# refresh-bio/colord

Measured on AMD Instinct MI355X. Metric: input Gbases/s + archive size vs ref, ONT 50 Gb at 1/2/4/8 MI355X, higher is better.
Workload: dtype u64

## Files before the change

colord_amd/_native.py:

```python
from __future__ import annotations
import ctypes as C
import os

os.environ.setdefault("GPU_MAX_HW_QUEUES", "32")
_HERE = os.path.dirname(os.path.abspath(__file__))
LIB_PATH = os.environ.get("COLORD_HIP_LIBRARY") or os.path.join(_HERE, "libcolord_hip.so")

CL_OK, CL_E_INVALID, CL_E_HIP, CL_E_CAPACITY, CL_E_NOMEM, CL_E_UNSUPPORTED = 0, -1, -2, -3, -4, -5


class ColordHipError(RuntimeError):
    def __init__(self, status, msg):
        super().__init__(f"colord_hip error {status}: {msg}")
        self.status = status


class QualParams(C.Structure):
    _fields_ = [("mode", C.c_int32), ("source", C.c_int32), ("level", C.c_int32), ("n_fwd", C.c_uint32), ("fwd", C.c_uint32 * 8),
                ("n_rev", C.c_uint32), ("rev", C.c_uint32 * 8)]


class KmerStats(C.Structure):
    _fields_ = [("n_reads", C.c_uint64), ("tot_kmers", C.c_uint64), ("n_unique", C.c_uint64),
                ("n_unique_counted", C.c_uint64), ("total_count_filtered", C.c_uint64)]
# ... 46 lines not shown
    "cl_kmer_count_filter": (C.c_int32, [_P, _P, C.c_uint64, C.c_uint32, C.c_uint32, C.c_uint32, C.POINTER(_P), C.POINTER(KmerStats)]),
    "cl_kmer_set_create": (C.c_int32, [_P, _P, _P, C.c_uint64, C.c_uint32, C.POINTER(_P)]),
    "cl_kmer_set_free": (None, [_P]),
    "cl_kmer_set_size": (C.c_uint64, [_P]),
    "cl_kmer_set_keys": (_P, [_P]),
    "cl_kmer_set_counts": (_P, [_P]),
    "cl_kmer_set_check": (C.c_int32, [_P, _P, _P, C.c_uint64, _P]),
    "cl_accepted_kmers": (C.c_int32, [_P, _P, _P, C.c_uint32, C.c_uint32, C.POINTER(_P)]),
    "cl_kmer_lists_free": (None, [_P]),
    "cl_kmer_lists_reads": (C.c_uint32, [_P]),
    "cl_kmer_lists_total": (C.c_uint64, [_P]),
    "cl_kmer_lists_offsets": (_P, [_P]),
    "cl_kmer_lists_kmers": (_P, [_P]),
    "cl_kmer_lists_ids": (_P, [_P]),
    "cl_kmer_lists_pos": (_P, [_P]),
    "cl_ref_accept": (C.c_int32, [C.c_uint32, C.c_uint32, C.c_uint32, C.c_double, _P]),
    "cl_index_build": (C.c_int32, [_P, _P, _P, _P, C.c_uint32, C.c_uint32, C.POINTER(_P)]),
    "cl_index_entries_of": (C.c_int32, [_P, _P, _P, C.c_uint32, _P, _P, C.c_uint64, C.POINTER(C.c_uint64), _P, C.POINTER(C.c_uint32)]),
    "cl_index_build_pairs": (C.c_int32, [_P, _P, _P, _P, C.c_uint64, _P, C.c_uint32, C.c_uint32, C.c_uint32, C.c_uint32, C.POINTER(_P)]),
    "cl_index_free": (None, [_P]),
    "cl_index_n_refs": (C.c_uint32, [_P]),
    "cl_index_entries": (C.c_uint64, [_P]),
    "cl_index_ref_rank": (_P, [_P]),
    "cl_candidates": (C.c_int32, [_P, _P, _P, C.c_uint32, _P, _P, _P]),
    "cl_candidates_common": (C.c_int32, [_P, _P, _P, C.c_uint32, _P, _P, _P, _P, C.c_uint64, C.POINTER(C.c_uint64)]),
    "cl_qual_coder_create": (C.c_int32, [_P, C.POINTER(QualParams), C.POINTER(_P)]),
    "cl_qual_coder_ctx": (_P, [_P]),
    "cl_qual_coder_free": (None, [_P]),
    "cl_qual_encode": (C.c_int32, [_P, _P, _P, _P, _P, _P, _P, C.c_uint32, _P, C.c_uint64, _P, C.POINTER(C.c_uint64)]),
    "cl_anchor_candidates": (C.c_int32, [_P, _P, _P, _P, _P, C.c_uint32, C.c_uint32, C.c_double, C.c_double, C.c_double, C.c_uint32, C.POINTER(_P)]),
    "cl_anchor_candidates_hifi": (C.c_int32, [_P, _P, _P, _P, _P, C.c_uint32, C.c_uint32, C.c_double, C.c_double, C.c_double, C.c_uint32, C.c_uint32, C.c_uint32, _P, _P, C.POINTER(_P)]),
    "cl_anchors_free": (None, [_P]),
    "cl_anchors_total": (C.c_uint64, [_P]),
    "cl_anchors_n_cands": (_P, [_P]),
    "cl_anchors_cands": (_P, [_P]),
    "cl_anchors_cand_offsets": (_P, [_P]),
    "cl_anchors_data": (_P, [_P]),
    "cl_encode_plain": (C.c_int32, [_P, _P, _P, C.c_uint64, _P, _P, C.POINTER(C.c_uint64)]),
    "cl_reads_select": (C.c_int32, [_P, _P, _P, C.POINTER(_P)]),
    "cl_reads_from_arena": (C.c_int32, [_P, _P, _P, _P, C.c_uint32, C.POINTER(_P)]),
    "cl_estimator_logs": (C.c_int32, [_P, _P, _P, C.c_uint64, _P]),
    "cl_es_flags": (C.c_int32, [_P, _P, _P, _P, _P, _P]),
    "cl_id_coder_create": (C.c_int32, [C.c_int32, C.POINTER(_P)]),
    "cl_id_coder_free": (None, [_P]),
    "cl_id_coder_error": (C.c_char_p, [_P]),
    "cl_id_encode_part": (C.c_int32, [_P, _P, _P, _P, C.c_uint32, _P, C.c_uint64, C.POINTER(C.c_uint64)]),
    "cl_compress_shard": (C.c_int32, [_P, C.POINTER(CompressParams), _P, _P, _P, _P, C.c_uint32, _P, C.c_uint32, _P, _P, _P, C.c_uint64, _P, _P, C.c_uint64, _P,
                                      C.POINTER(CompressInfo)]),
    "cl_candidates_at": (C.c_int32, [_P, _P, _P, _P, C.c_uint32, _P, _P, _P]),
    "cl_compressor_create": (C.c_int32, [_P, _P, C.POINTER(CompressParams), C.POINTER(QualParams), C.POINTER(Exchange), C.c_uint64, C.POINTER(_P)]),
    "cl_compressor_free": (None, [_P]),
    "cl_compressor_count_add": (C.c_int32, [_P, _P]),
    "cl_compressor_count_finish": (C.c_int32, [_P, C.POINTER(KmerStats)]),
    "cl_compressor_refs_add": (C.c_int32, [_P, _P]),
    "cl_compressor_refs_finish": (C.c_int32, [_P]),
    "cl_compressor_encode": (C.c_int32, [_P, _P, _P, _P, _P, C.c_uint32, _P, C.c_uint32, _P, C.c_uint64, _P, _P, C.c_uint64, _P, C.POINTER(CompressInfo)]),
    "cl_compressor_genome_add": (C.c_int32, [_P, _P]),
    "cl_compressor_pseudo_reads": (C.c_int32, [_P, _P]),
    "cl_genome_encode": (C.c_int32, [_P, _P, C.c_uint32, _P, C.c_uint64, C.POINTER(C.c_uint64)]),
    "cl_genome_decode": (C.c_int32, [_P, C.c_uint64, C.c_uint32, _P, C.c_uint64, _P, C.POINTER(C.c_uint64)]),
    "cl_genome_md5": (C.c_int32, [_P, _P, C.c_uint32, _P]),
    "cl_compressor_prepare": (C.c_int32, [_P, _P, _P, C.c_uint32]),
    "cl_compressor_prepare_parts": (C.c_int32, [_P, _P, _P, C.c_uint32, _P, C.c_uint32, _P, _P]),
    "cl_compressor_info": (C.c_int32, [_P, C.POINTER(KmerStats), C.POINTER(C.c_uint64), C.POINTER(C.c_uint64), C.POINTER(C.c_uint64), C.POINTER(C.c_uint32), C.POINTER(C.c_uint32)]),
    "cl_dna_decoder_create": (C.c_int32, [C.c_uint32, C.c_int32, C.c_uint32, C.c_uint32, C.c_int32, C.c_uint32, C.c_double, C.POINTER(_P)]),
    "cl_dna_decoder_free": (None, [_P]),
    "cl_dna_decoder_error": (C.c_char_p, [_P]),
    "cl_dna_decoder_add_ref": (C.c_int32, [_P, _P, C.c_uint32]),
    "cl_dna_decoder_new_domain": (C.c_int32, [_P]),
    "cl_dna_decode_part": (C.c_int32, [_P, _P, C.c_uint64, C.c_uint32, _P, C.c_uint64, _P, C.POINTER(C.c_uint64)]),
    "cl_qual_decoder_create": (C.c_int32, [C.POINTER(QualParams), C.POINTER(_P)]),
    "cl_qual_decoder_free": (None, [_P]),
    "cl_qual_decoder_new_domain": (C.c_int32, [_P]),
    "cl_qual_decode_part": (C.c_int32, [_P, _P, C.c_uint64, _P, _P, C.c_uint32, _P]),
    "cl_id_decoder_create": (C.c_int32, [C.c_int32, C.POINTER(_P)]),
    "cl_id_decoder_free": (None, [_P]),
    "cl_id_decode_part": (C.c_int32, [_P, _P, C.c_uint64, C.c_uint32, _P, C.c_uint64, _P, _P, C.POINTER(C.c_uint64)]),
    "cl_encode_reads": (C.c_int32, [_P, _P, _P, _P, C.c_uint32, C.c_uint32, C.c_uint32, C.c_uint32, C.c_double, _P, C.c_uint32, _P, C.c_uint64, _P, _P, C.POINTER(C.c_uint64)]),
    "cl_dna_coder_create": (C.c_int32, [_P, C.c_uint32, C.c_int32, C.c_uint32, C.POINTER(_P)]),
    "cl_dna_coder_free": (None, [_P]),
    "cl_dna_encode": (C.c_int32, [_P, _P, _P, _P, _P, _P, C.c_uint32, _P, C.c_uint32, _P, C.c_uint64, _P, C.POINTER(C.c_uint64)]),
    "cl_sort_u64": (C.c_int32, [_P, _P, C.c_uint64, C.c_uint32, C.c_uint32]),
    "cl_sort_u64_u32": (C.c_int32, [_P, _P, _P, C.c_uint64, C.c_uint32, C.c_uint32]),
}

_lib = None


def load():
    global _lib
    if _lib is None:
        if not os.path.exists(LIB_PATH):
            raise ColordHipError(CL_E_HIP, f"{LIB_PATH} is missing: run `make -C colord_amd/csrc` "
                                 "(or __graft_entry__.build()); there is no CPU fallback")
        lib = C.CDLL(LIB_PATH)
        for name, (res, args) in _SIG.items():
            fn = getattr(lib, name)
            fn.restype, fn.argtypes = res, args
        _lib = lib
    return _lib


def exported_names():
    return sorted(_SIG)
```

colord_amd/csrc/capi.hip:

```cpp
#include "common.hpp"
#include "objects.hpp"
#include <cmath>
#include <random>

extern "C" cl_status cl_ctx_create(int device, cl_ctx** out)
{
	if (!out) return CL_E_INVALID;
	*out = nullptr;
	int n = 0;
	hipError_t e = hipGetDeviceCount(&n);
	if (e != hipSuccess || n <= 0) { fprintf(stderr, "colord_hip: no HIP device available (%s)\n", hipGetErrorString(e)); return CL_E_HIP; }
	if (device < 0 || device >= n) return CL_E_INVALID;
	if (hipSetDevice(device) != hipSuccess) return CL_E_HIP;
	cl_ctx* c = new cl_ctx(device);
	if (hipStreamCreateWithFlags(&c->stream, hipStreamNonBlocking) != hipSuccess) { cl_ctx_destroy(c); return CL_E_HIP; }
	hipDeviceProp_t p;
	if (hipGetDeviceProperties(&p, device) == hipSuccess) c->n_cu = p.multiProcessorCount;
	*out = c;
	return CL_OK;
}
void cl_ctx_set_priority(cl_ctx* c, int level, int role)
{
	if (!c) return;
	(void)hipSetDevice(c->device);
// ... 63 lines not shown
	return n;
}
extern "C" void cl_ctx_destroy(cl_ctx* c)
{
	if (!c) return;
	for (cl_ctx* l : c->lanes) cl_ctx_destroy(l);
	c->lanes.clear();
	if (c->prep) { cl_ctx_destroy(c->prep); c->prep = nullptr; }
	if (c->qprep) { cl_ctx_destroy(c->qprep); c->qprep = nullptr; }
	(void)hipSetDevice(c->device);
	cl_ctx_drain(c);
	for (auto& kv : c->scan_ctl) if (kv.second.p) c->pool.put(kv.second.p, kv.second.got, c->pool_id);
	c->scan_ctl.clear();
	c->pool.drop_owner(c->pool_id);
	for (auto& p : c->pending) { (void)hipEventDestroy(p.second.first); (void)hipEventDestroy(p.second.second); }
	for (auto e : c->ev_pool) (void)hipEventDestroy(e);
	if (c->stream) (void)hipStreamDestroy(c->stream);
	for (std::atomic<hipStream_t>* s : { &c->side, &c->side2, &c->side3 }) if (hipStream_t x = s->load()) (void)hipStreamDestroy(x);
	if (c->inv_tab) (void)hipFree(c->inv_tab);
	if (c->slots_h) (void)hipHostFree(c->slots_h);
	const int dev = c->device;
	delete c;
	cl_device_pool_release(dev);
}
extern "C" const char* cl_last_error(const cl_ctx* c) { return c ? c->err.c_str() : "null context"; }
extern "C" void* cl_ctx_stream(cl_ctx* c) { return c ? (void*)c->stream : nullptr; }
extern "C" void cl_ctx_set_timing(cl_ctx* c, int on) { if (c) c->timing = on != 0; }
extern "C" cl_status cl_ctx_last_kernel_ms(const cl_ctx* c, const char* kernel, double* ms, uint32_t* launches)
{
	if (!c || !kernel) return CL_E_INVALID;
	auto it = c->times.find(kernel);
	if (it == c->times.end()) { if (ms) *ms = 0; if (launches) *launches = 0; return CL_E_INVALID; }
	if (ms) *ms = it->second.ms;
	if (launches) *launches = it->second.launches;
	return CL_OK;
}

extern "C" cl_status cl_ctx_kernel_times(cl_ctx* c, char* buf, uint64_t cap, uint64_t* needed)
{
	if (!c) return CL_E_INVALID;
	cl_timing_collect(c);
	std::string out;
	for (auto& kv : c->times) out += kv.first + "\t" + std::to_string(kv.second.ms) + "\t" + std::to_string(kv.second.launches) + "\t" + std::to_string(kv.second.bytes) + "\t" + std::to_string(kv.second.cells) + "\n";
	if (needed) *needed = out.size() + 1;
	if (!buf || cap < out.size() + 1) return CL_E_CAPACITY;
	memcpy(buf, out.c_str(), out.size() + 1);
	c->times.clear();
	return CL_OK;
}

extern "C" cl_status cl_ref_accept(uint32_t n_reads, uint32_t n_pseudo, uint32_t range, double exponent, uint8_t* h_out)
{
	if (!h_out || range == 0) return CL_E_INVALID;
	std::mt19937 mt;
	std::uniform_real_distribution<double> dist(0.0, 1.0);
	for (uint64_t i = 0; i < (uint64_t)n_reads + n_pseudo; ++i)
	{
		if (i < n_pseudo) { h_out[i] = 1; continue; }
		uint32_t range_no = (uint32_t)((i - n_pseudo) / range);
		double p = std::pow(1.0 / (range_no + 1ul), exponent);
		h_out[i] = dist(mt) <= p;
	}
	return CL_OK;
}

extern "C" cl_status cl_sort_u64(cl_ctx* ctx, uint64_t* d_keys, uint64_t n, uint32_t begin_bit, uint32_t end_bit)
{
	if (!ctx || (!d_keys && n)) return cl_fail(ctx, CL_E_INVALID, "cl_sort_u64: null argument");
	HIP_TRY(ctx, hipSetDevice(ctx->device));
	cl_timing_begin(ctx);
	cl_status s = dev_sort_pairs(ctx, d_keys, nullptr, n, begin_bit, end_bit);
	cl_timing_collect(ctx);
	return s;
}
extern "C" cl_status cl_sort_u64_u32(cl_ctx* ctx, uint64_t* d_keys, uint32_t* d_vals, uint64_t n, uint32_t begin_bit, uint32_t end_bit)
{
	if (!ctx || ((!d_keys || !d_vals) && n)) return cl_fail(ctx, CL_E_INVALID, "cl_sort_u64_u32: null argument");
	HIP_TRY(ctx, hipSetDevice(ctx->device));
	cl_timing_begin(ctx);
	cl_status s = dev_sort_pairs(ctx, d_keys, d_vals, n, begin_bit, end_bit);
	cl_timing_collect(ctx);
	return s;
}
```

colord_amd/csrc/sort.hip:

```cpp
#include "common.hpp"
#include <string>

namespace {
constexpr uint32_t ST = 256;
constexpr uint32_t SI = 16;
constexpr uint32_t STILE = ST * SI;

template<typename K, uint32_t DB, uint32_t G>
__global__ __launch_bounds__(ST) void k_sort_hist(const K* __restrict__ keys, uint64_t n, uint32_t shift,
                                                  uint32_t* __restrict__ hist, uint32_t nb)
{
	constexpr uint32_t ND = 1u << DB;
	constexpr uint32_t ROW = G > 1 ? ND + 1 : ND;
	__shared__ uint32_t h[G * ROW];
	for (uint32_t i = threadIdx.x; i < G * ROW; i += ST) h[i] = 0;
	__syncthreads();
	const uint32_t tile0 = blockIdx.x * G;
	for (uint32_t g = 0; g < G && tile0 + g < nb; ++g)
	{
		const uint64_t base = (uint64_t)(tile0 + g) * STILE;
#pragma unroll
		for (uint32_t i = 0; i < SI; ++i)
		{
			uint64_t idx = base + (uint64_t)i * ST + threadIdx.x;
			if (idx < n) atomicAdd(&h[g * ROW + ((uint32_t)(keys[idx] >> shift) & (ND - 1))], 1u);
		}
	}
	__syncthreads();
	for (uint32_t i = threadIdx.x; i < G * ND; i += ST)
	{
		const uint32_t g = i % G, d = i / G;
		if (tile0 + g < nb) hist[(uint64_t)d * nb + tile0 + g] = h[g * ROW + d];
	}
}

template<typename K, bool HAS_V, uint32_t DB>
__global__ __launch_bounds__(ST) void k_sort_scatter(const K* __restrict__ kin, const uint32_t* __restrict__ vin,
                                                     K* __restrict__ kout, uint32_t* __restrict__ vout,
                                                     uint64_t n, uint32_t shift, const uint32_t* __restrict__ offs, uint32_t nb)
{
	constexpr uint32_t ND = 1u << DB, PER = ND / ST;
	__shared__ uint32_t wh[4][ND];
	__shared__ uint32_t lstart[ND + 1];
	__shared__ uint32_t gdelta[ND];
	__shared__ uint32_t wtot[4];
	__shared__ K skey[STILE];
	__shared__ uint32_t sval[HAS_V ? STILE : 1];
	const uint32_t w = threadIdx.x >> 6, lane = threadIdx.x & 63;
	for (uint32_t i = threadIdx.x; i < 4 * ND; i += ST) (&wh[0][0])[i] = 0;
	__syncthreads();

	const uint64_t tbase = (uint64_t)blockIdx.x * STILE, wbase = tbase + (uint64_t)w * (64 * SI);
	K key[SI]; uint32_t rank[SI]; uint32_t val[HAS_V ? SI : 1];
	const uint64_t lt = (1ULL << lane) - 1;
	uint32_t goff[PER];
#pragma unroll
	for (uint32_t k = 0; k < PER; ++k) goff[k] = offs[(uint64_t)(threadIdx.x * PER + k) * nb + blockIdx.x];
#pragma unroll
	for (uint32_t r = 0; r < SI; ++r)
	{
		uint64_t idx = wbase + (uint64_t)r * 64 + lane;
		key[r] = idx < n ? kin[idx] : (K)0;
		if (HAS_V) val[r] = idx < n ? vin[idx] : 0u;
	}
#pragma unroll
	for (uint32_t r = 0; r < SI; ++r)
	{
		uint64_t idx = wbase + (uint64_t)r * 64 + lane;
		bool valid = idx < n;
		uint32_t d = (uint32_t)(key[r] >> shift) & (ND - 1);
		uint64_t peers = __ballot(valid);
#pragma unroll
		for (uint32_t b = 0; b < DB; ++b)
		{
			bool bit = (d >> b) & 1u;
			uint64_t m = __ballot(valid && bit);
			peers &= bit ? m : ~m;
		}
		uint32_t prior = valid ? wh[w][d] : 0u;
		rank[r] = prior + (uint32_t)__popcll(peers & lt);
		__builtin_amdgcn_wave_barrier();
		if (valid && (peers & lt) == 0) wh[w][d] = prior + (uint32_t)__popcll(peers);
		__builtin_amdgcn_wave_barrier();
	}
	__syncthreads();
	{
		uint32_t c[PER][4], tot[PER], mine = 0;
#pragma unroll
		for (uint32_t k = 0; k < PER; ++k)
		{
			const uint32_t d = threadIdx.x * PER + k;
			c[k][0] = wh[0][d]; c[k][1] = wh[1][d]; c[k][2] = wh[2][d]; c[k][3] = wh[3][d];
			tot[k] = c[k][0] + c[k][1] + c[k][2] + c[k][3]; mine += tot[k];
		}
		uint32_t incl = mine;
#pragma unroll
		for (uint32_t o = 1; o < 64; o <<= 1) { const uint32_t t = __shfl_up(incl, o, 64); if (lane >= o) incl += t; }
		if (lane == 63) wtot[w] = incl;
		__syncthreads();
		uint32_t ls = incl - mine;
		for (uint32_t i = 0; i < w; ++i) ls += wtot[i];
#pragma unroll
		for (uint32_t k = 0; k < PER; ++k)
		{
			const uint32_t d = threadIdx.x * PER + k;
			lstart[d] = ls;
			if (d == ND - 1) lstart[ND] = ls + tot[k];
			gdelta[d] = goff[k] - ls;
			wh[0][d] = ls; wh[1][d] = ls + c[k][0]; wh[2][d] = ls + c[k][0] + c[k][1]; wh[3][d] = ls + c[k][0] + c[k][1] + c[k][2];
			ls += tot[k];
		}
	}
	__syncthreads();
#pragma unroll
	for (uint32_t r = 0; r < SI; ++r)
	{
		uint64_t idx = wbase + (uint64_t)r * 64 + lane;
		if (idx < n)
		{
			uint32_t d = (uint32_t)(key[r] >> shift) & (ND - 1);
			uint32_t lp = wh[w][d] + rank[r];
			skey[lp] = key[r];
			if (HAS_V) sval[lp] = val[r];
		}
	}
	__syncthreads();
	const uint32_t tile_n = lstart[ND];
	for (uint32_t j = threadIdx.x; j < tile_n; j += ST)
	{
		const K k = skey[j];
		const uint32_t pos = gdelta[(uint32_t)(k >> shift) & (ND - 1)] + j;
		kout[pos] = k;
		if (HAS_V) vout[pos] = sval[j];
	}
}

template<typename K, uint32_t DB>
cl_status sort_pass(cl_ctx* ctx, const K* kin, const uint32_t* vin, K* kout, uint32_t* vout, uint64_t n, uint32_t shift, uint32_t* hist, uint32_t nb)
{
	static const std::string kt = sizeof(K) == 8 ? "unsigned long" : "unsigned int", db = std::to_string(DB) + "u";
	constexpr uint32_t G = DB == 8 ? 16 : 4; const bool grouped = nb >= 4096;
	static const std::string n_hist1 = "k_sort_hist<" + kt + ", " + db + ", 1u>", n_histg = "k_sort_hist<" + kt + ", " + db + ", " + std::to_string(G) + "u>", n_sv = "k_sort_scatter<" + kt + ", true, " + db + ">", n_sk = "k_sort_scatter<" + kt + ", false, " + db + ">";
	if (grouped) LAUNCHB_NAMED(ctx, n_histg.c_str(), n * sizeof(K), (k_sort_hist<K, DB, G>), (nb + G - 1) / G, ST, kin, n, shift, hist, nb);
	else LAUNCHB_NAMED(ctx, n_hist1.c_str(), n * sizeof(K), (k_sort_hist<K, DB, 1>), nb, ST, kin, n, shift, hist, nb);
	HIP_TRY(ctx, hipGetLastError());
	CL_TRY(dev_exclusive_scan_u32(ctx, hist, (uint64_t)(1u << DB) * nb, nullptr));
	if (vin) LAUNCHB_NAMED(ctx, n_sv.c_str(), n * (2 * sizeof(K) + 8), (k_sort_scatter<K, true, DB>), nb, ST, kin, vin, kout, vout, n, shift, (const uint32_t*)hist, nb);
	else LAUNCHB_NAMED(ctx, n_sk.c_str(), n * 2 * sizeof(K), (k_sort_scatter<K, false, DB>), nb, ST, kin, (const uint32_t*)nullptr, kout, (uint32_t*)nullptr, n, shift, (const uint32_t*)hist, nb);
	HIP_TRY(ctx, hipGetLastError());
	return CL_OK;
}

template<typename K>
cl_status sort_impl(cl_ctx* ctx, K* d_keys, uint32_t* d_vals, uint64_t n, uint32_t begin_bit, uint32_t end_bit, DevBuf<K>* swap_k = nullptr, DevBuf<uint32_t>* swap_v = nullptr)
{
	if (n <= 1 || end_bit <= begin_bit) return CL_OK;
	if (n >= (1ULL << 32)) return cl_fail(ctx, CL_E_UNSUPPORTED, "radix sort: n must be < 2^32 per call");
	const uint32_t nb = grid_for(n, STILE);
	const uint32_t bits = end_bit - begin_bit;
	const uint32_t n_pass_real = (bits + 7) / 8 == (bits + 9) / 10 ? (bits + 7) / 8 : (bits + 9) / 10;
	const uint32_t db_hi = (bits + n_pass_real - 1) / n_pass_real;
	const bool third = (n_pass_real & 1) && n_pass_real > 1 && n * (sizeof(K) + (d_vals ? 4 : 0)) <= (2ull << 30);
	const uint32_t n_pass = third ? n_pass_real : (n_pass_real + 1) & ~1u;
	DevBuf<K> ktmp, ktmp2; DEV_ALLOC(ctx, ktmp, n);
	DevBuf<uint32_t> vtmp, vtmp2; if (d_vals) DEV_ALLOC(ctx, vtmp, n);
	if (n_pass & 1) { DEV_ALLOC(ctx, ktmp2, n); if (d_vals) DEV_ALLOC(ctx, vtmp2, n); }
	DevBuf<uint32_t> hist; DEV_ALLOC(ctx, hist, (uint64_t)(1u << std::max(8u, db_hi)) * nb);
	K* kin = d_keys; uint32_t* vin = d_vals;
	uint32_t pass = 0;
	for (uint32_t shift = begin_bit; shift < end_bit; ++pass)
	{
		K* kout; uint32_t* vout;
		if (n_pass & 1) { kout = pass == 0 ? ktmp2.p : (pass & 1) ? ktmp.p : d_keys; vout = pass == 0 ? vtmp2.p : (pass & 1) ? vtmp.p : d_vals; }
		else { kout = (pass & 1) ? d_keys : ktmp.p; vout = (pass & 1) ? d_vals : vtmp.p; }
		const uint32_t left = end_bit - shift, passes_left = n_pass_real - pass;
		const uint32_t db = std::max(8u, (left + passes_left - 1) / passes_left);
		const uint32_t use = std::min(db, 10u);
		if (use == 10) CL_TRY((sort_pass<K, 10>(ctx, kin, vin, kout, vout, n, shift, hist.p, nb)));
		else if (use == 9) CL_TRY((sort_pass<K, 9>(ctx, kin, vin, kout, vout, n, shift, hist.p, nb)));
		else CL_TRY((sort_pass<K, 8>(ctx, kin, vin, kout, vout, n, shift, hist.p, nb)));
		shift += use;
		kin = kout; vin = vout;
	}
	if (kin != d_keys && swap_k && kin == ktmp.p && (!d_vals || (swap_v && vin == vtmp.p)))
	{
		std::swap(*swap_k, ktmp);
		if (d_vals) std::swap(*swap_v, vtmp);
	}
	else if (kin != d_keys)
	{
		HIP_TRY(ctx, hipMemcpyAsync(d_keys, kin, n * sizeof(K), hipMemcpyDeviceToDevice, cl_launch_stream(ctx)));
		if (d_vals) HIP_TRY(ctx, hipMemcpyAsync(d_vals, vin, n * 4, hipMemcpyDeviceToDevice, cl_launch_stream(ctx)));
	}
	HIP_TRY(ctx, hipStreamSynchronize(cl_launch_stream(ctx)));
	return CL_OK;
}
}

cl_status dev_sort_pairs(cl_ctx* ctx, uint64_t* d_keys, uint32_t* d_vals, uint64_t n, uint32_t begin_bit, uint32_t end_bit)
{
	return sort_impl<uint64_t>(ctx, d_keys, d_vals, n, begin_bit, end_bit);
}
cl_status dev_sort_pairs_swap(cl_ctx* ctx, DevBuf<uint64_t>& keys, DevBuf<uint32_t>& vals, uint64_t n, uint32_t begin_bit, uint32_t end_bit)
{
	if (keys.n != n || vals.n != n) return sort_impl<uint64_t>(ctx, keys.p, vals.p, n, begin_bit, end_bit);
	return sort_impl<uint64_t>(ctx, keys.p, vals.p, n, begin_bit, end_bit, &keys, &vals);
}
cl_status dev_sort_keys32_pairs(cl_ctx* ctx, uint32_t* d_keys, uint32_t* d_vals, uint64_t n, uint32_t begin_bit, uint32_t end_bit)
{
	return sort_impl<uint32_t>(ctx, d_keys, d_vals, n, begin_bit, end_bit);
}
cl_status dev_sort_keys32_pairs_swap(cl_ctx* ctx, DevBuf<uint32_t>& keys, DevBuf<uint32_t>& vals, uint64_t n, uint32_t begin_bit, uint32_t end_bit)
{
	if (keys.n != n || vals.n != n) return sort_impl<uint32_t>(ctx, keys.p, vals.p, n, begin_bit, end_bit);
	return sort_impl<uint32_t>(ctx, keys.p, vals.p, n, begin_bit, end_bit, &keys, &vals);
}
```

colord_amd/device.py:

```python
from __future__ import annotations
import ctypes as C
import numpy as np
import torch
from . import _native as N


def _check(ctx, st):
    if ctx is not None and getattr(ctx, "timing", False):
        for n, (ms, k, b, cells) in ctx.kernel_times().items():
            a = ctx.acc.setdefault(n, [0.0, 0, 0.0, 0.0])
            a[0] += ms
            a[1] += k
            a[2] += b
            a[3] += cells
    if st != N.CL_OK:
        msg = N.load().cl_last_error(ctx.h).decode() if ctx is not None and ctx.h else ""
        raise N.ColordHipError(st, msg)


def _view(ptr, n, dtype, device):
    out = torch.empty(int(n), dtype=dtype, device=device)
    if n:
        torch.cuda.synchronize(device)
        rc = _hip().hipMemcpy(C.c_void_p(out.data_ptr()), C.c_void_p(ptr), C.c_size_t(int(n) * out.element_size()), 3)
# ... 226 lines not shown
        n = reads.n_reads
        pb = np.ascontiguousarray(np.asarray([0, n] if pack_bounds is None else pack_bounds, dtype=np.uint32))
        off = torch.empty(n + 1, dtype=torch.int64, device=self.device)
        nt = torch.empty(max(n, 1), dtype=torch.int32, device=self.device)
        need = C.c_uint64(0)
        cap = int(reads.total_bases) + 16 * n + 4096
        for _ in range(2):
            es = torch.empty(max(cap, 1), dtype=torch.uint8, device=self.device)
            st = self.lib.cl_encode_reads(self.h, reads.h, refs.h, anchors.h, anchors.c, anchor_len, min_part_alt, max_rec, cost_mult,
                                          pb.ctypes.data, len(pb) - 1, es.data_ptr(), cap, off.data_ptr(), nt.data_ptr(), C.byref(need))
            if st == N.CL_E_CAPACITY and need.value > cap:
                cap = need.value
                continue
            _check(self, st)
            break
        return es[:need.value], off, nt[:n]

    def es_flags(self, reads: "Reads", es: torch.Tensor, es_off: torch.Tensor, base_off: torch.Tensor) -> torch.Tensor:
        flags = torch.empty(max(int(reads.total_bases), 1), dtype=torch.uint8, device=self.device)
        _check(self, self.lib.cl_es_flags(self.h, reads.h, es.contiguous().data_ptr() if es.numel() else None, es_off.contiguous().data_ptr(),
                                          base_off.contiguous().data_ptr(), flags.data_ptr()))
        return flags[:int(reads.total_bases)]

    def estimator_logs(self, count: torch.Tensor, total: torch.Tensor) -> torch.Tensor:
        count, total = count.contiguous(), total.contiguous()
        assert count.dtype == torch.int32 and total.dtype == torch.int32 and count.numel() == total.numel()
        out = torch.empty(count.numel(), dtype=torch.float64, device=self.device)
        _check(self, self.lib.cl_estimator_logs(self.h, count.data_ptr(), total.data_ptr(), count.numel(), out.data_ptr()))
        return out

    def compress_shard(self, reads: "Reads", params: dict, part_bounds, pack_bounds, dna: "DnaCoder", qual: "QualCoder | None" = None,
                       quals: torch.Tensor | None = None, base_off: torch.Tensor | None = None):
        import numpy as np
        P = N.CompressParams()
        for k_, v in params.items():
            setattr(P, k_, v)
        pb = np.ascontiguousarray(np.asarray(part_bounds, dtype=np.uint32)); kb = np.ascontiguousarray(np.asarray(pack_bounds, dtype=np.uint32))
        npart = len(pb) - 1
        dcap = int(reads.total_bases) + 64 * npart + 4096
        dout = torch.empty(dcap, dtype=torch.uint8, device=self.device)
        dsz = np.zeros(max(npart, 1), np.uint64)
        qout, qsz, qcap = None, np.zeros(max(npart, 1), np.uint64), 0
        if qual is not None:
            qcap = int(int(reads.total_bases) * 1.35) + 64 * npart + 4096
            qout = torch.empty(qcap, dtype=torch.uint8, device=self.device)
        info = N.CompressInfo()
        _check(self, self.lib.cl_compress_shard(self.h, C.byref(P), reads.h, quals.data_ptr() if qual is not None else None,
                                                base_off.contiguous().data_ptr() if qual is not None else None,
                                                pb.ctypes.data, npart, kb.ctypes.data, len(kb) - 1, dna.h, qual.h if qual is not None else None,
                                                dout.data_ptr(), dcap, dsz.ctypes.data, qout.data_ptr() if qout is not None else None, qcap, qsz.ctypes.data, C.byref(info)))
        if qual is not None and qual.ctx is not self:
            _check(qual.ctx, N.CL_OK)
        inf = {n_: getattr(info, n_) for n_, _ in N.CompressInfo._fields_ if n_ != "pad"}
        return dout[:inf["dna_bytes"]], dsz[:npart], (qout[:inf["qual_bytes"]] if qout is not None else None), qsz[:npart], inf

    def compressor(self, params: dict, qual_params=None, qual_ctx: "Context | None" = None, exchange=None, expected_bases: int = 0) -> "Compressor":
        P = N.CompressParams()
        for k_, v in params.items():
            setattr(P, k_, v)
        Q = None
        if qual_params is not None:
            mode, source, level, fwd, rev = qual_params
            Q = N.QualParams(mode=mode, source=source, level=level, n_fwd=len(fwd), n_rev=len(rev))
            for i, v in enumerate(fwd):
                Q.fwd[i] = v
            for i, v in enumerate(rev):
                Q.rev[i] = v
        h = N._P()
        _check(self, self.lib.cl_compressor_create(self.h, qual_ctx.h if qual_ctx is not None else None, C.byref(P), C.byref(Q) if Q is not None else None,
                                                   C.byref(exchange.c_struct) if exchange is not None else None, int(expected_bases), C.byref(h)))
        return Compressor(self, h, qual_ctx, Q is not None, exchange)

    def dna_coder(self, max_alt_refs: int, level: int, start_read_id: int = 0) -> "DnaCoder":
        h = N._P()
        _check(self, self.lib.cl_dna_coder_create(self.h, max_alt_refs, level, start_read_id, C.byref(h)))
        return DnaCoder(self, h)

    def sort_u64(self, keys: torch.Tensor, vals: torch.Tensor | None = None, begin_bit=0, end_bit=64):
        if vals is None:
            _check(self, self.lib.cl_sort_u64(self.h, keys.data_ptr(), keys.numel(), begin_bit, end_bit))
        else:
            _check(self, self.lib.cl_sort_u64_u32(self.h, keys.data_ptr(), vals.data_ptr(), keys.numel(), begin_bit, end_bit))


class _Obj:
    _free = None

    def __init__(self, ctx, h):
        self.ctx, self.h = ctx, h

    def free(self):
        if self.h:
            getattr(self.ctx.lib, self._free)(self.h)
            self.h = None

    def _arr(self, getter, n, dtype):
        ptr = getattr(self.ctx.lib, getter)(self.h)
        return _view(ptr, n, dtype, self.ctx.device)


class Reads(_Obj):
    _free = "cl_reads_free"

    @property
    def n_reads(self): return self.ctx.lib.cl_reads_count(self.h)
    @property
    def total_bases(self): return self.ctx.lib.cl_reads_total_bases(self.h)
    @property
    def total_words(self): return self.ctx.lib.cl_reads_total_words(self.h)
    def packed(self): return self._arr("cl_reads_packed", self.total_words + 1, torch.int64)
    def invalid(self): return self._arr("cl_reads_invalid", self.total_words + 1, torch.int32)
    def word_offsets(self): return self._arr("cl_reads_word_offsets", self.n_reads + 1, torch.int64)
    def lengths(self): return self._arr("cl_reads_lengths", self.n_reads, torch.int32)
    def has_n(self): return self._arr("cl_reads_has_n", self.n_reads, torch.uint8)

    def compact(self, i: int) -> bytes:
        buf = np.zeros(1 << 20, np.uint8)
        n = C.c_uint64(0)
        st = self.ctx.lib.cl_reads_compact(self.ctx.h, self.h, i, buf.ctypes.data, buf.size, C.byref(n))
        if st == N.CL_E_CAPACITY:
            buf = np.zeros(n.value, np.uint8)
            st = self.ctx.lib.cl_reads_compact(self.ctx.h, self.h, i, buf.ctypes.data, buf.size, C.byref(n))
        _check(self.ctx, st)
        return bytes(buf[:n.value])


class KmerSet(_Obj):
    _free = "cl_kmer_set_free"

    @property
    def size(self): return self.ctx.lib.cl_kmer_set_size(self.h)
    def keys(self): return self._arr("cl_kmer_set_keys", self.size, torch.int64)
    def counts(self): return self._arr("cl_kmer_set_counts", self.size, torch.int32)

    def check(self, kmers: torch.Tensor) -> torch.Tensor:
        out = torch.empty(kmers.numel(), dtype=torch.uint8, device=self.ctx.device)
        _check(self.ctx, self.ctx.lib.cl_kmer_set_check(self.ctx.h, self.h, kmers.data_ptr(), kmers.numel(), out.data_ptr()))
        return out


class KmerLists(_Obj):
    _free = "cl_kmer_lists_free"

    @property
    def n_reads(self): return self.ctx.lib.cl_kmer_lists_reads(self.h)
    @property
    def total(self): return self.ctx.lib.cl_kmer_lists_total(self.h)
    def offsets(self): return self._arr("cl_kmer_lists_offsets", self.n_reads + 1, torch.int64)
    def kmers(self): return self._arr("cl_kmer_lists_kmers", self.total, torch.int64)
    def ids(self): return self._arr("cl_kmer_lists_ids", self.total, torch.int32)
    def pos(self): return self._arr("cl_kmer_lists_pos", self.total, torch.int32)


class Index(_Obj):
    _free = "cl_index_free"

    @property
    def n_refs(self): return self.ctx.lib.cl_index_n_refs(self.h)
    @property
    def entries(self): return self.ctx.lib.cl_index_entries(self.h)


class QualCoder(_Obj):
    _free = "cl_qual_coder_free"

    def encode(self, reads: "Reads", quals: torch.Tensor, qual_off: torch.Tensor, part_bounds, flags: torch.Tensor | None = None):
# ... 111 lines not shown
```

include/colord_hip.h:

```cpp
#ifndef COLORD_HIP_H
#define COLORD_HIP_H
#include <stdint.h>
#include <stddef.h>

#ifdef __cplusplus
extern "C" {
#endif

typedef int32_t cl_status;
enum {
	CL_OK = 0,
	CL_E_INVALID = -1,
	CL_E_HIP = -2,
	CL_E_CAPACITY = -3,
	CL_E_NOMEM = -4,
	CL_E_UNSUPPORTED = -5
};

typedef struct cl_ctx cl_ctx;
typedef struct cl_reads cl_reads;
typedef struct cl_kmer_set cl_kmer_set;
typedef struct cl_kmer_lists cl_kmer_lists;
typedef struct cl_index cl_index;

// ... 122 lines not shown
cl_status cl_reads_from_arena(cl_ctx* ctx, const uint64_t* d_packed, const uint32_t* d_inv, const uint32_t* d_lens, uint32_t n_reads, cl_reads** out);

typedef struct cl_id_coder cl_id_coder;
cl_status cl_id_coder_create(int32_t header_mode, cl_id_coder** out);
void cl_id_coder_free(cl_id_coder* c);
const char* cl_id_coder_error(const cl_id_coder* c);
cl_status cl_id_encode_part(cl_id_coder* c, const uint8_t* h_ids, const uint64_t* h_off, const uint8_t* h_plus, uint32_t n,
                            uint8_t* h_out, uint64_t cap, uint64_t* n_out);

typedef struct {
	uint32_t k, f, ci, cs, c;
	uint32_t anchor_len, min_part_alt, max_rec, min_anchors;
	int32_t level, source;
	int32_t sparse;
	double sparse_g, sparse_exponent;
	double cost_mult, frac_always, frac_min, max_matches_mult;
} cl_compress_params;
typedef struct {
	uint64_t n_reads, n_bases, tot_kmers, n_kept_kmers, n_refs, n_anchors, tuple_bytes, dna_bytes, qual_bytes;
	uint32_t sparse_range, pad;
} cl_compress_info;
cl_status cl_compress_shard(cl_ctx* ctx, const cl_compress_params* params, const cl_reads* reads, const uint8_t* d_quals, const uint64_t* d_base_off,
                            const uint32_t* h_part_bounds, uint32_t n_parts, const uint32_t* h_pack_bounds, uint32_t n_packs,
                            cl_dna_coder* dna, cl_qual_coder* qual,
                            uint8_t* d_dna_out, uint64_t dna_cap, uint64_t* h_dna_part_sizes,
                            uint8_t* d_qual_out, uint64_t qual_cap, uint64_t* h_qual_part_sizes, cl_compress_info* info);

typedef struct cl_compressor cl_compressor;
typedef struct {
	void* user;
	uint32_t rank, world;
	cl_status (*all_gather_host)(void* user, const uint64_t* h_vals, uint32_t n, uint64_t* h_out);
	cl_status (*all_to_all_v)(void* user, const void* d_send, const uint64_t* h_send_bytes, void* d_recv, const uint64_t* h_recv_bytes);
	cl_status (*all_gather_v)(void* user, const void* d_send, uint64_t send_bytes, void* d_recv, const uint64_t* h_recv_bytes);
} cl_exchange;
cl_status cl_compressor_create(cl_ctx* ctx, cl_ctx* qual_ctx, const cl_compress_params* params, const cl_qual_params* qparams,
                               const cl_exchange* exchange, uint64_t expected_bases, cl_compressor** out);
void cl_compressor_free(cl_compressor* c);
cl_status cl_compressor_count_add(cl_compressor* c, const cl_reads* chunk);
cl_status cl_compressor_count_finish(cl_compressor* c, cl_kmer_stats* stats);
cl_status cl_compressor_refs_add(cl_compressor* c, const cl_reads* chunk);
cl_status cl_compressor_refs_finish(cl_compressor* c);
cl_status cl_compressor_encode(cl_compressor* c, const cl_reads* chunk, const uint8_t* d_quals, const uint64_t* d_base_off,
                               const uint32_t* h_part_bounds, uint32_t n_parts, const uint32_t* h_pack_bounds, uint32_t n_packs,
                               uint8_t* d_dna_out, uint64_t dna_cap, uint64_t* h_dna_part_sizes,
                               uint8_t* d_qual_out, uint64_t qual_cap, uint64_t* h_qual_part_sizes, cl_compress_info* info);
cl_status cl_compressor_genome_add(cl_compressor* c, const cl_reads* sequences);
cl_status cl_compressor_pseudo_reads(cl_compressor* c, const cl_reads* pseudo_reads);
cl_status cl_compressor_prepare(cl_compressor* c, const cl_reads* chunk, const uint32_t* h_pack_bounds, uint32_t n_packs);
cl_status cl_compressor_prepare_parts(cl_compressor* c, const cl_reads* chunk, const uint32_t* h_pack_bounds, uint32_t n_packs, const uint32_t* h_part_bounds, uint32_t n_parts,
                                      const uint8_t* d_quals, const uint64_t* d_base_off);
cl_status cl_compressor_info(const cl_compressor* c, cl_kmer_stats* stats, uint64_t* first_read, uint64_t* n_reads_total, uint64_t* mean_read_len,
                             uint32_t* sparse_range, uint32_t* n_refs_total);

cl_status cl_genome_encode(const uint8_t* h_codes, const uint64_t* h_off, uint32_t n_seqs, uint8_t* h_out, uint64_t cap, uint64_t* n_out);
cl_status cl_genome_decode(const uint8_t* h_in, uint64_t n_in, uint32_t n_seqs, uint8_t* h_codes, uint64_t cap, uint64_t* h_off, uint64_t* n_out);
cl_status cl_genome_md5(const uint8_t* h_codes, const uint64_t* h_off, uint32_t n_seqs, uint8_t* h_md5_16);

typedef struct cl_dna_decoder cl_dna_decoder;
typedef struct cl_qual_decoder cl_qual_decoder;
typedef struct cl_id_decoder cl_id_decoder;
cl_status cl_dna_decoder_create(uint32_t max_alt_refs, int32_t level, uint32_t start_read_id, uint32_t n_pseudo,
                                int32_t accept_all, uint32_t sparse_range, double sparse_exponent, cl_dna_decoder** out);
void cl_dna_decoder_free(cl_dna_decoder* d);
const char* cl_dna_decoder_error(const cl_dna_decoder* d);
cl_status cl_dna_decoder_add_ref(cl_dna_decoder* d, const uint8_t* h_codes, uint32_t len);
cl_status cl_dna_decoder_new_domain(cl_dna_decoder* d);
cl_status cl_dna_decode_part(cl_dna_decoder* d, const uint8_t* h_in, uint64_t n_in, uint32_t n_reads,
                             uint8_t* h_bases, uint64_t cap, uint64_t* h_off, uint64_t* n_out);
cl_status cl_qual_decoder_create(const cl_qual_params* params, cl_qual_decoder** out);
void cl_qual_decoder_free(cl_qual_decoder* q);
cl_status cl_qual_decoder_new_domain(cl_qual_decoder* q);
cl_status cl_qual_decode_part(cl_qual_decoder* q, const uint8_t* h_in, uint64_t n_in, const uint8_t* h_bases, const uint64_t* h_off,
                              uint32_t n_reads, uint8_t* h_quals);
cl_status cl_id_decoder_create(int32_t header_mode, cl_id_decoder** out);
void cl_id_decoder_free(cl_id_decoder* c);
cl_status cl_id_decode_part(cl_id_decoder* c, const uint8_t* h_in, uint64_t n_in, uint32_t n, uint8_t* h_ids, uint64_t cap,
                            uint64_t* h_off, uint8_t* h_plus, uint64_t* n_out);

cl_status cl_reads_compact(cl_ctx* ctx, const cl_reads* reads, uint32_t read, uint8_t* h_out, uint64_t cap, uint64_t* n_out);

cl_status cl_sort_u64(cl_ctx* ctx, uint64_t* d_keys, uint64_t n, uint32_t begin_bit, uint32_t end_bit);
cl_status cl_sort_u64_u32(cl_ctx* ctx, uint64_t* d_keys, uint32_t* d_vals, uint64_t n, uint32_t begin_bit, uint32_t end_bit);

#ifdef __cplusplus
}
#endif
#endif
```

Measured before the change: 2.801.

## Restructure radix sort histogram layout and scan into tile-major column scan

Histogram counts are now stored tile-major (one row of digit counts per tile), so the scatter kernel can load its offsets as one contiguous row. The histogram kernel aggregates per-wave digit matches with ballots, issuing one shared atomic per distinct digit per wave instead of one per key. The generic exclusive scan is replaced by a column scan that works directly on that layout, with a hierarchical sum/scan/add path for many tiles. The scatter kernel reuses a single shared buffer for keys and then values, which cuts shared memory per block. A u32-key sort entry point is also exposed. The costs are three small scan launches for large inputs and an extra barrier-separated phase for values.

```diff
diff --git a/colord_amd/_native.py b/colord_amd/_native.py
--- a/colord_amd/_native.py
+++ b/colord_amd/_native.py
@@ -152,6 +152,7 @@
     "cl_dna_encode": (C.c_int32, [_P, _P, _P, _P, _P, _P, C.c_uint32, _P, C.c_uint32, _P, C.c_uint64, _P, C.POINTER(C.c_uint64)]),
     "cl_sort_u64": (C.c_int32, [_P, _P, C.c_uint64, C.c_uint32, C.c_uint32]),
     "cl_sort_u64_u32": (C.c_int32, [_P, _P, _P, C.c_uint64, C.c_uint32, C.c_uint32]),
+    "cl_sort_u32_u32": (C.c_int32, [_P, _P, _P, C.c_uint64, C.c_uint32, C.c_uint32]),
 }
 
 _lib = None
diff --git a/colord_amd/csrc/capi.hip b/colord_amd/csrc/capi.hip
--- a/colord_amd/csrc/capi.hip
+++ b/colord_amd/csrc/capi.hip
@@ -169,3 +169,12 @@
 	cl_timing_collect(ctx);
 	return s;
 }
+extern "C" cl_status cl_sort_u32_u32(cl_ctx* ctx, uint32_t* d_keys, uint32_t* d_vals, uint64_t n, uint32_t begin_bit, uint32_t end_bit)
+{
+	if (!ctx || (!d_keys && n)) return cl_fail(ctx, CL_E_INVALID, "cl_sort_u32_u32: null argument");
+	HIP_TRY(ctx, hipSetDevice(ctx->device));
+	cl_timing_begin(ctx);
+	cl_status s = dev_sort_keys32_pairs(ctx, d_keys, d_vals, n, begin_bit, end_bit);
+	cl_timing_collect(ctx);
+	return s;
+}
diff --git a/colord_amd/csrc/sort.hip b/colord_amd/csrc/sort.hip
--- a/colord_amd/csrc/sort.hip
+++ b/colord_amd/csrc/sort.hip
@@ -5,57 +5,177 @@
 constexpr uint32_t ST = 256;
 constexpr uint32_t SI = 16;
 constexpr uint32_t STILE = ST * SI;
-
-template<typename K, uint32_t DB, uint32_t G>
-__global__ __launch_bounds__(ST) void k_sort_hist(const K* __restrict__ keys, uint64_t n, uint32_t shift,
-                                                  uint32_t* __restrict__ hist, uint32_t nb)
+constexpr uint32_t SCAN_BATCH = 16;
+constexpr uint32_t SCAN_DIRECT = 64;
+
+template<uint32_t PER> __device__ inline void row_load(const uint32_t* p, uint32_t (&v)[PER]) { __builtin_memcpy(v, __builtin_assume_aligned(p, 4 * PER), 4 * PER); }
+template<uint32_t PER> __device__ inline void row_store(uint32_t* p, const uint32_t (&v)[PER]) { __builtin_memcpy(__builtin_assume_aligned(p, 4 * PER), v, 4 * PER); }
+
+template<uint32_t DB> __device__ inline uint64_t digit_peers(uint32_t d, bool valid)
+{
+	uint64_t peers = __ballot(valid);
+#pragma unroll
+	for (uint32_t b = 0; b < DB; ++b)
+	{
+		const bool bit = (d >> b) & 1u;
+		const uint64_t m = __ballot(valid && bit);
+		peers &= bit ? m : ~m;
+	}
+	return peers;
+}
+
+template<typename K, uint32_t DB>
+__global__ __launch_bounds__(ST) void k_sort_hist(const K* __restrict__ keys, uint64_t n, uint32_t shift, uint32_t* __restrict__ counts)
 {
 	constexpr uint32_t ND = 1u << DB;
-	constexpr uint32_t ROW = G > 1 ? ND + 1 : ND;
-	__shared__ uint32_t h[G * ROW];
-	for (uint32_t i = threadIdx.x; i < G * ROW; i += ST) h[i] = 0;
-	__syncthreads();
-	const uint32_t tile0 = blockIdx.x * G;
-	for (uint32_t g = 0; g < G && tile0 + g < nb; ++g)
-	{
-		const uint64_t base = (uint64_t)(tile0 + g) * STILE;
-#pragma unroll
-		for (uint32_t i = 0; i < SI; ++i)
-		{
-			uint64_t idx = base + (uint64_t)i * ST + threadIdx.x;
-			if (idx < n) atomicAdd(&h[g * ROW + ((uint32_t)(keys[idx] >> shift) & (ND - 1))], 1u);
-		}
-	}
-	__syncthreads();
-	for (uint32_t i = threadIdx.x; i < G * ND; i += ST)
-	{
-		const uint32_t g = i % G, d = i / G;
-		if (tile0 + g < nb) hist[(uint64_t)d * nb + tile0 + g] = h[g * ROW + d];
+	__shared__ uint32_t h[ND];
+	for (uint32_t i = threadIdx.x; i < ND; i += ST) h[i] = 0;
+	const uint64_t base = (uint64_t)blockIdx.x * STILE;
+	const uint64_t lt = (1ULL << (threadIdx.x & 63)) - 1;
+	K key[SI];
+#pragma unroll
+	for (uint32_t i = 0; i < SI; ++i)
+	{
+		const uint64_t idx = base + (uint64_t)i * ST + threadIdx.x;
+		key[i] = idx < n ? keys[idx] : (K)0;
+	}
+	__syncthreads();
+#pragma unroll
+	for (uint32_t i = 0; i < SI; ++i)
+	{
+		const bool valid = base + (uint64_t)i * ST + threadIdx.x < n;
+		const uint32_t d = (uint32_t)(key[i] >> shift) & (ND - 1);
+		const uint64_t peers = digit_peers<DB>(d, valid);
+		if (valid && (peers & lt) == 0) atomicAdd(&h[d], (uint32_t)__popcll(peers));
+	}
+	__syncthreads();
+	uint32_t* row = counts + (uint64_t)blockIdx.x * ND;
+	for (uint32_t i = threadIdx.x; i < ND; i += ST) row[i] = h[i];
+}
+
+template<uint32_t DB>
+__global__ __launch_bounds__(ST) void k_sort_colsum(const uint32_t* __restrict__ counts, uint32_t nb, uint32_t gt, uint32_t* __restrict__ gsum)
+{
+	constexpr uint32_t ND = 1u << DB, PER = ND / ST;
+	const uint32_t t0 = blockIdx.x * gt, t1 = min(nb, t0 + gt);
+	uint32_t s[PER] = {};
+	for (uint32_t t = t0; t < t1; t += SCAN_BATCH)
+	{
+		uint32_t v[SCAN_BATCH][PER];
+#pragma unroll
+		for (uint32_t j = 0; j < SCAN_BATCH; ++j)
+		{
+			if (t + j < t1) row_load<PER>(counts + (uint64_t)(t + j) * ND + threadIdx.x * PER, v[j]);
+			else for (uint32_t k = 0; k < PER; ++k) v[j][k] = 0;
+		}
+#pragma unroll
+		for (uint32_t j = 0; j < SCAN_BATCH; ++j)
+			for (uint32_t k = 0; k < PER; ++k) s[k] += v[j][k];
+	}
+	row_store<PER>(gsum + (uint64_t)blockIdx.x * ND + threadIdx.x * PER, s);
+}
+
+template<uint32_t DB>
+__global__ __launch_bounds__(4 * ST) void k_sort_colscan(uint32_t* __restrict__ tab, uint32_t rows)
+{
+	constexpr uint32_t ND = 1u << DB, PER = ND / ST;
+	__shared__ uint32_t part[4][ND];
+	__shared__ uint32_t wtot[4][4];
+	const uint32_t s = threadIdx.x / ST, t = threadIdx.x % ST, w = t >> 6, lane = threadIdx.x & 63;
+	const uint32_t q = (rows + 3) / 4, r0 = min(rows, s * q), r1 = min(rows, r0 + q);
+	uint32_t sum[PER] = {};
+	for (uint32_t r = r0; r < r1; r += SCAN_BATCH)
+	{
+		uint32_t v[SCAN_BATCH][PER];
+#pragma unroll
+		for (uint32_t j = 0; j < SCAN_BATCH; ++j)
+		{
+			if (r + j < r1) row_load<PER>(tab + (uint64_t)(r + j) * ND + t * PER, v[j]);
+			else for (uint32_t k = 0; k < PER; ++k) v[j][k] = 0;
+		}
+#pragma unroll
+		for (uint32_t j = 0; j < SCAN_BATCH; ++j)
+			for (uint32_t k = 0; k < PER; ++k) sum[k] += v[j][k];
+	}
+#pragma unroll
+	for (uint32_t k = 0; k < PER; ++k) part[s][t * PER + k] = sum[k];
+	__syncthreads();
+	uint32_t run[PER], tot[PER], mine = 0;
+#pragma unroll
+	for (uint32_t k = 0; k < PER; ++k)
+	{
+		const uint32_t d = t * PER + k;
+		run[k] = 0; tot[k] = 0;
+		for (uint32_t i = 0; i < 4; ++i) { if (i < s) run[k] += part[i][d]; tot[k] += part[i][d]; }
+		mine += tot[k];
+	}
+	uint32_t incl = mine;
+#pragma unroll
+	for (uint32_t o = 1; o < 64; o <<= 1) { const uint32_t x = __shfl_up(incl, o, 64); if (lane >= o) incl += x; }
+	if (lane == 63) wtot[s][w] = incl;
+	__syncthreads();
+	uint32_t ls = incl - mine;
+	for (uint32_t i = 0; i < w; ++i) ls += wtot[s][i];
+#pragma unroll
+	for (uint32_t k = 0; k < PER; ++k) { run[k] += ls; ls += tot[k]; }
+	for (uint32_t r = r0; r < r1; r += SCAN_BATCH)
+	{
+		uint32_t v[SCAN_BATCH][PER];
+#pragma unroll
+		for (uint32_t j = 0; j < SCAN_BATCH; ++j)
+			if (r + j < r1) row_load<PER>(tab + (uint64_t)(r + j) * ND + t * PER, v[j]);
+#pragma unroll
+		for (uint32_t j = 0; j < SCAN_BATCH; ++j)
+			if (r + j < r1)
+			{
+				row_store<PER>(tab + (uint64_t)(r + j) * ND + t * PER, run);
+				for (uint32_t k = 0; k < PER; ++k) run[k] += v[j][k];
+			}
+	}
+}
+
+template<uint32_t DB>
+__global__ __launch_bounds__(ST) void k_sort_coladd(uint32_t* __restrict__ counts, uint32_t nb, uint32_t gt, const uint32_t* __restrict__ gsum)
+{
+	constexpr uint32_t ND = 1u << DB, PER = ND / ST;
+	const uint32_t t0 = blockIdx.x * gt, t1 = min(nb, t0 + gt);
+	uint32_t run[PER];
+	row_load<PER>(gsum + (uint64_t)blockIdx.x * ND + threadIdx.x * PER, run);
+	for (uint32_t t = t0; t < t1; t += SCAN_BATCH)
+	{
+		uint32_t v[SCAN_BATCH][PER];
+#pragma unroll
+		for (uint32_t j = 0; j < SCAN_BATCH; ++j)
+			if (t + j < t1) row_load<PER>(counts + (uint64_t)(t + j) * ND + threadIdx.x * PER, v[j]);
+#pragma unroll
+		for (uint32_t j = 0; j < SCAN_BATCH; ++j)
+			if (t + j < t1)
+			{
+				row_store<PER>(counts + (uint64_t)(t + j) * ND + threadIdx.x * PER, run);
+				for (uint32_t k = 0; k < PER; ++k) run[k] += v[j][k];
+			}
 	}
 }
 
 template<typename K, bool HAS_V, uint32_t DB>
 __global__ __launch_bounds__(ST) void k_sort_scatter(const K* __restrict__ kin, const uint32_t* __restrict__ vin,
                                                      K* __restrict__ kout, uint32_t* __restrict__ vout,
-                                                     uint64_t n, uint32_t shift, const uint32_t* __restrict__ offs, uint32_t nb)
+                                                     uint64_t n, uint32_t shift, const uint32_t* __restrict__ offs)
 {
 	constexpr uint32_t ND = 1u << DB, PER = ND / ST;
 	__shared__ uint32_t wh[4][ND];
-	__shared__ uint32_t lstart[ND + 1];
 	__shared__ uint32_t gdelta[ND];
 	__shared__ uint32_t wtot[4];
-	__shared__ K skey[STILE];
-	__shared__ uint32_t sval[HAS_V ? STILE : 1];
+	__shared__ K sbuf[STILE];
 	const uint32_t w = threadIdx.x >> 6, lane = threadIdx.x & 63;
 	for (uint32_t i = threadIdx.x; i < 4 * ND; i += ST) (&wh[0][0])[i] = 0;
 	__syncthreads();
 
 	const uint64_t tbase = (uint64_t)blockIdx.x * STILE, wbase = tbase + (uint64_t)w * (64 * SI);
-	K key[SI]; uint32_t rank[SI]; uint32_t val[HAS_V ? SI : 1];
+	K key[SI]; uint32_t lp[SI]; uint32_t val[HAS_V ? SI : 1];
 	const uint64_t lt = (1ULL << lane) - 1;
 	uint32_t goff[PER];
-#pragma unroll
-	for (uint32_t k = 0; k < PER; ++k) goff[k] = offs[(uint64_t)(threadIdx.x * PER + k) * nb + blockIdx.x];
+	row_load<PER>(offs + (uint64_t)blockIdx.x * ND + threadIdx.x * PER, goff);
 #pragma unroll
 	for (uint32_t r = 0; r < SI; ++r)
 	{
@@ -69,16 +189,9 @@
 		uint64_t idx = wbase + (uint64_t)r * 64 + lane;
 		bool valid = idx < n;
 		uint32_t d = (uint32_t)(key[r] >> shift) & (ND - 1);
-		uint64_t peers = __ballot(valid);
-#pragma unroll
-		for (uint32_t b = 0; b < DB; ++b)
-		{
-			bool bit = (d >> b) & 1u;
-			uint64_t m = __ballot(valid && bit);
-			peers &= bit ? m : ~m;
-		}
+		const uint64_t peers = digit_peers<DB>(d, valid);
 		uint32_t prior = valid ? wh[w][d] : 0u;
-		rank[r] = prior + (uint32_t)__popcll(peers & lt);
+		lp[r] = prior + (uint32_t)__popcll(peers & lt);
 		__builtin_amdgcn_wave_barrier();
 		if (valid && (peers & lt) == 0) wh[w][d] = prior + (uint32_t)__popcll(peers);
 		__builtin_amdgcn_wave_barrier();
@@ -104,8 +217,6 @@
 		for (uint32_t k = 0; k < PER; ++k)
 		{
 			const uint32_t d = threadIdx.x * PER + k;
-			lstart[d] = ls;
-			if (d == ND - 1) lstart[ND] = ls + tot[k];
 			gdelta[d] = goff[k] - ls;
 			wh[0][d] = ls; wh[1][d] = ls + c[k][0]; wh[2][d] = ls + c[k][0] + c[k][1]; wh[3][d] = ls + c[k][0] + c[k][1] + c[k][2];
 			ls += tot[k];
@@ -119,34 +230,73 @@
 		if (idx < n)
 		{
 			uint32_t d = (uint32_t)(key[r] >> shift) & (ND - 1);
-			uint32_t lp = wh[w][d] + rank[r];
-			skey[lp] = key[r];
-			if (HAS_V) sval[lp] = val[r];
-		}
-	}
-	__syncthreads();
-	const uint32_t tile_n = lstart[ND];
-	for (uint32_t j = threadIdx.x; j < tile_n; j += ST)
-	{
-		const K k = skey[j];
-		const uint32_t pos = gdelta[(uint32_t)(k >> shift) & (ND - 1)] + j;
-		kout[pos] = k;
-		if (HAS_V) vout[pos] = sval[j];
-	}
+			lp[r] += wh[w][d];
+			sbuf[lp[r]] = key[r];
+		}
+	}
+	__syncthreads();
+	const uint32_t tile_n = (uint32_t)min((uint64_t)STILE, n - tbase);
+	uint32_t pos[HAS_V ? SI : 1];
+#pragma unroll
+	for (uint32_t i = 0; i < SI; ++i)
+	{
+		const uint32_t j = i * ST + threadIdx.x;
+		if (j < tile_n)
+		{
+			const K k = sbuf[j];
+			const uint32_t p = gdelta[(uint32_t)(k >> shift) & (ND - 1)] + j;
+			kout[p] = k;
+			if (HAS_V) pos[i] = p;
+		}
+	}
+	if (HAS_V)
+	{
+		uint32_t* sv = reinterpret_cast<uint32_t*>(sbuf);
+		__syncthreads();
+#pragma unroll
+		for (uint32_t r = 0; r < SI; ++r)
+			if (wbase + (uint64_t)r * 64 + lane < n) sv[lp[r]] = val[r];
+		__syncthreads();
+#pragma unroll
+		for (uint32_t i = 0; i < SI; ++i)
+		{
+			const uint32_t j = i * ST + threadIdx.x;
+			if (j < tile_n) vout[pos[i]] = sv[j];
+		}
+	}
+}
+
+inline uint32_t scan_group(uint32_t nb)
+{
+	if (nb <= SCAN_DIRECT) return 1;
+	uint32_t gt = 1;
+	while ((uint64_t)gt * gt < nb) gt <<= 1;
+	return gt;
 }
 
 template<typename K, uint32_t DB>
-cl_status sort_pass(cl_ctx* ctx, const K* kin, const uint32_t* vin, K* kout, uint32_t* vout, uint64_t n, uint32_t shift, uint32_t* hist, uint32_t nb)
-{
+cl_status sort_pass(cl_ctx* ctx, const K* kin, const uint32_t* vin, K* kout, uint32_t* vout, uint64_t n, uint32_t shift, uint32_t* counts, uint32_t* gsum, uint32_t nb)
+{
+	constexpr uint32_t ND = 1u << DB;
 	static const std::string kt = sizeof(K) == 8 ? "unsigned long" : "unsigned int", db = std::to_string(DB) + "u";
-	constexpr uint32_t G = DB == 8 ? 16 : 4; const bool grouped = nb >= 4096;
-	static const std::string n_hist1 = "k_sort_hist<" + kt + ", " + db + ", 1u>", n_histg = "k_sort_hist<" + kt + ", " + db + ", " + std::to_string(G) + "u>", n_sv = "k_sort_scatter<" + kt + ", true, " + db + ">", n_sk = "k_sort_scatter<" + kt + ", false, " + db + ">";
-	if (grouped) LAUNCHB_NAMED(ctx, n_histg.c_str(), n * sizeof(K), (k_sort_hist<K, DB, G>), (nb + G - 1) / G, ST, kin, n, shift, hist, nb);
-	else LAUNCHB_NAMED(ctx, n_hist1.c_str(), n * sizeof(K), (k_sort_hist<K, DB, 1>), nb, ST, kin, n, shift, hist, nb);
+	static const std::string n_hist = "k_sort_hist<" + kt + ", " + db + ">", n_sv = "k_sort_scatter<" + kt + ", true, " + db + ">", n_sk = "k_sort_scatter<" + kt + ", false, " + db + ">";
+	static const std::string n_csum = "k_sort_colsum<" + db + ">", n_cscan = "k_sort_colscan<" + db + ">", n_cadd = "k_sort_coladd<" + db + ">";
+	LAUNCHB_NAMED(ctx, n_hist.c_str(), n * sizeof(K) + (uint64_t)nb * ND * 4, (k_sort_hist<K, DB>), nb, ST, kin, n, shift, counts);
 	HIP_TRY(ctx, hipGetLastError());
-	CL_TRY(dev_exclusive_scan_u32(ctx, hist, (uint64_t)(1u << DB) * nb, nullptr));
-	if (vin) LAUNCHB_NAMED(ctx, n_sv.c_str(), n * (2 * sizeof(K) + 8), (k_sort_scatter<K, true, DB>), nb, ST, kin, vin, kout, vout, n, shift, (const uint32_t*)hist, nb);
-	else LAUNCHB_NAMED(ctx, n_sk.c_str(), n * 2 * sizeof(K), (k_sort_scatter<K, false, DB>), nb, ST, kin, (const uint32_t*)nullptr, kout, (uint32_t*)nullptr, n, shift, (const uint32_t*)hist, nb);
+	const uint32_t gt = scan_group(nb);
+	if (gt == 1) LAUNCHB_NAMED(ctx, n_cscan.c_str(), (uint64_t)nb * ND * 8, (k_sort_colscan<DB>), 1, 4 * ST, counts, nb);
+	else
+	{
+		const uint32_t ng = (nb + gt - 1) / gt;
+		LAUNCHB_NAMED(ctx, n_csum.c_str(), (uint64_t)nb * ND * 4, (k_sort_colsum<DB>), ng, ST, (const uint32_t*)counts, nb, gt, gsum);
+		HIP_TRY(ctx, hipGetLastError());
+		LAUNCHB_NAMED(ctx, n_cscan.c_str(), (uint64_t)ng * ND * 8, (k_sort_colscan<DB>), 1, 4 * ST, gsum, ng);
+		HIP_TRY(ctx, hipGetLastError());
+		LAUNCHB_NAMED(ctx, n_cadd.c_str(), (uint64_t)nb * ND * 8, (k_sort_coladd<DB>), ng, ST, counts, nb, gt, (const uint32_t*)gsum);
+	}
+	HIP_TRY(ctx, hipGetLastError());
+	if (vin) LAUNCHB_NAMED(ctx, n_sv.c_str(), n * (2 * sizeof(K) + 8), (k_sort_scatter<K, true, DB>), nb, ST, kin, vin, kout, vout, n, shift, (const uint32_t*)counts);
+	else LAUNCHB_NAMED(ctx, n_sk.c_str(), n * 2 * sizeof(K), (k_sort_scatter<K, false, DB>), nb, ST, kin, (const uint32_t*)nullptr, kout, (uint32_t*)nullptr, n, shift, (const uint32_t*)counts);
 	HIP_TRY(ctx, hipGetLastError());
 	return CL_OK;
 }
@@ -165,7 +315,9 @@
 	DevBuf<K> ktmp, ktmp2; DEV_ALLOC(ctx, ktmp, n);
 	DevBuf<uint32_t> vtmp, vtmp2; if (d_vals) DEV_ALLOC(ctx, vtmp, n);
 	if (n_pass & 1) { DEV_ALLOC(ctx, ktmp2, n); if (d_vals) DEV_ALLOC(ctx, vtmp2, n); }
-	DevBuf<uint32_t> hist; DEV_ALLOC(ctx, hist, (uint64_t)(1u << std::max(8u, db_hi)) * nb);
+	const uint32_t gt = scan_group(nb), ng = (nb + gt - 1) / gt;
+	DevBuf<uint32_t> hist; DEV_ALLOC(ctx, hist, (uint64_t)(1u << std::max(8u, db_hi)) * (nb + (gt > 1 ? ng : 0)));
+	uint32_t* gsum = hist.p + (uint64_t)(1u << std::max(8u, db_hi)) * nb;
 	K* kin = d_keys; uint32_t* vin = d_vals;
 	uint32_t pass = 0;
 	for (uint32_t shift = begin_bit; shift < end_bit; ++pass)
@@ -176,9 +328,9 @@
 		const uint32_t left = end_bit - shift, passes_left = n_pass_real - pass;
 		const uint32_t db = std::max(8u, (left + passes_left - 1) / passes_left);
 		const uint32_t use = std::min(db, 10u);
-		if (use == 10) CL_TRY((sort_pass<K, 10>(ctx, kin, vin, kout, vout, n, shift, hist.p, nb)));
-		else if (use == 9) CL_TRY((sort_pass<K, 9>(ctx, kin, vin, kout, vout, n, shift, hist.p, nb)));
-		else CL_TRY((sort_pass<K, 8>(ctx, kin, vin, kout, vout, n, shift, hist.p, nb)));
+		if (use == 10) CL_TRY((sort_pass<K, 10>(ctx, kin, vin, kout, vout, n, shift, hist.p, gsum, nb)));
+		else if (use == 9) CL_TRY((sort_pass<K, 9>(ctx, kin, vin, kout, vout, n, shift, hist.p, gsum, nb)));
+		else CL_TRY((sort_pass<K, 8>(ctx, kin, vin, kout, vout, n, shift, hist.p, gsum, nb)));
 		shift += use;
 		kin = kout; vin = vout;
 	}
diff --git a/colord_amd/device.py b/colord_amd/device.py
--- a/colord_amd/device.py
+++ b/colord_amd/device.py
@@ -332,6 +332,9 @@
         else:
             _check(self, self.lib.cl_sort_u64_u32(self.h, keys.data_ptr(), vals.data_ptr(), keys.numel(), begin_bit, end_bit))
 
+    def sort_u32(self, keys: torch.Tensor, vals: torch.Tensor | None = None, begin_bit=0, end_bit=32):
+        _check(self, self.lib.cl_sort_u32_u32(self.h, keys.data_ptr(), vals.data_ptr() if vals is not None else None, keys.numel(), begin_bit, end_bit))
+
 
 class _Obj:
     _free = None
diff --git a/include/colord_hip.h b/include/colord_hip.h
--- a/include/colord_hip.h
+++ b/include/colord_hip.h
@@ -228,6 +228,7 @@
 
 cl_status cl_sort_u64(cl_ctx* ctx, uint64_t* d_keys, uint64_t n, uint32_t begin_bit, uint32_t end_bit);
 cl_status cl_sort_u64_u32(cl_ctx* ctx, uint64_t* d_keys, uint32_t* d_vals, uint64_t n, uint32_t begin_bit, uint32_t end_bit);
+cl_status cl_sort_u32_u32(cl_ctx* ctx, uint32_t* d_keys, uint32_t* d_vals, uint64_t n, uint32_t begin_bit, uint32_t end_bit);
 
 #ifdef __cplusplus
 }
```

After: 2.757 (median of 2 runs). 1.6% lower.
